# nrlugg/fenix

Measured on AMD Instinct MI355X. Metric: vectors/sec + %HBM roofline, 10M×768 f32 L2 kNN k=100 at 1/2/4/8 GPU, higher is better.
Workload: dtype f32; 1 GPU; 10Mx768 f32 L2 kNN k=100, single query, per GPU; rows_per_gpu=10000000, total_rows=10000000, d=768, k=100, queries=1, metric=l2, parallelism=row-shard x1, one process per GPU

## Files before the change

fenix_amd/_lib.py:

```python

from __future__ import annotations

import contextlib
import ctypes
import hashlib
import os
import threading
from typing import Iterator

HERE = os.path.dirname(os.path.abspath(__file__))
LIB_PATH = os.environ.get("FENIX_AMD_LIB") or os.path.join(HERE, "lib", "libfenix_knn.so")

DTYPE_F32 = 0
DTYPE_F16 = 1
DTYPE_QU8 = 2
METRIC_L2 = 0
METRIC_IP = 1
METRIC_COS = 2

METRICS = {
    "l2": METRIC_L2,
    "euclidean": METRIC_L2,
    "inner_product": METRIC_IP,
    "dot": METRIC_IP,
    "cosine": METRIC_COS,
}

SYMBOLS = (
    "fx_version",
    "fx_last_error",
    "fx_device_count",
    "fx_max_k",
    "fx_knn_workspace_bytes",
    "fx_knn_workspace_bytes_img8",
    "fx_knn_search",
    "fx_knn_scan",
    "fx_knn_reduce",
    "fx_filter_image_bytes",
    "fx_filter_image",
    "fx_filter_image_used",
    "fx_knn_scan_img",
    "fx_knn_search_img",
    "fx_filter_image8_bytes",
    "fx_filter_image8",
    "fx_knn_scan_img8",
    "fx_knn_search_img8",
    "fx_knn_reduce_img8",
    "fx_filter_image8_typed",
    "fx_filter_image8_perm",
    "fx_knn_filter_counts",
    "fx_knn_filter_state",
    "fx_knn_distances",
    "fx_topk_merge_workspace_bytes",
    "fx_topk_merge",
    "fx_fill_normal",
    "fx_row_sqnorms",
    "fx_code_assign_workspace_bytes",
    "fx_code_assign",
    "fx_kmeans_step_workspace_bytes",
    "fx_kmeans_step",
    "fx_code_assign_ex",
    "fx_kmeans_step_ex",
    "fx_code_probe_workspace_bytes",
    "fx_code_probe",
    "fx_code_mask",
    "fx_code_qmask_workspace_bytes",
    "fx_code_qmask",
    "fx_knn_search_rows_workspace_bytes",
    "fx_knn_search_rows",
    "fx_mask_compact_workspace_bytes",
    "fx_mask_compact",
    "fx_pred_limits",
    "fx_pred_eval",
    "fx_knn_search_ex_workspace_bytes",
    "fx_knn_search_ex",
    "fx_knn_search_shards_workspace_bytes",
    "fx_knn_search_shards",
    "fx_knn_distances_ex",
    "fx_filter_image8_ex",
    "fx_knn_scan_img8_ex",
    "fx_knn_reduce_img8_ex",
    "fx_knn_search_img8_ex",
    "fx_qmask_words",
    "fx_qmask_pack",
    "fx_qmask_filter_used",
    "fx_knn_scan_qmask_ex",
    "fx_knn_reduce_qmask_ex",
    "fx_knn_search_qmask_ex",
    "fx_comm_init_all",
    "fx_comm_destroy",
    "fx_allgather_topk",
    "fx_set_option",
    "fx_get_option",
    "fx_host_sync_count",
)

OPTIONS = ("batched", "batch_min_queries", "batch_cap", "batch_sample_ratio", "force_fallback",
           "scan_interleave", "q8_dma", "filter_image", "batch_ub_test", "single_query_image",
           "i8_max_k", "img6", "img8", "i8_sample_ratio", "i8_grow_ratio", "select_prune",
           "scan_stream", "filter_hold", "qu8_batch_min_work", "qmask_batch_min_ratio",
           "device_filter_min_rows")

_lock = threading.Lock()
_lib = None


class Corpus(ctypes.Structure):

    _fields_ = [
        ("data", ctypes.c_void_p),
        ("dtype", ctypes.c_int),
        ("n", ctypes.c_int64),
        ("d", ctypes.c_int64),
        ("row_base", ctypes.c_int64),
        ("scale", ctypes.c_float),
        ("zero_point", ctypes.c_int32),
    ]


class PredColumn(ctypes.Structure):

    _fields_ = [
        ("values", ctypes.c_void_p),
        ("valid", ctypes.c_void_p),
        ("dtype", ctypes.c_int32),
        ("reserved", ctypes.c_int32),
    ]


class PredOp(ctypes.Structure):

    _fields_ = [
        ("op", ctypes.c_int32),
        ("column", ctypes.c_int32),
        ("imm", ctypes.c_int64),
        ("set_offset", ctypes.c_int32),
        ("set_length", ctypes.c_int32),
    ]


class FenixHipError(RuntimeError):
    """A HIP runtime failure inside the kNN engine."""


def load() -> ctypes.CDLL:
    global _lib
    with _lock:
        if _lib is not None:
            return _lib
        if not os.path.exists(LIB_PATH):
            raise ImportError(
                f"fenix_amd HIP library not built: {LIB_PATH} is missing "
                "(run __graft_entry__.build() or `make -C fenix_amd/csrc`)"
            )
        L = ctypes.CDLL(LIB_PATH)
        i64, sz, vp, ci = ctypes.c_int64, ctypes.c_size_t, ctypes.c_void_p, ctypes.c_int
        L.fx_version.argtypes = []
        L.fx_version.restype = ci
        L.fx_last_error.argtypes = []
        L.fx_last_error.restype = ctypes.c_char_p
        L.fx_device_count.argtypes = [ctypes.POINTER(ci)]
        L.fx_device_count.restype = ci
        L.fx_max_k.argtypes = []
        L.fx_max_k.restype = i64
        L.fx_knn_workspace_bytes.argtypes = [i64, i64, ci, i64, i64, ctypes.POINTER(sz)]
        L.fx_knn_workspace_bytes.restype = ci
        L.fx_knn_workspace_bytes_img8.argtypes = [i64, i64, ci, i64, i64, ci, ctypes.POINTER(sz)]
        L.fx_knn_workspace_bytes_img8.restype = ci
        L.fx_knn_search.argtypes = [vp, ci, i64, i64, i64, vp, i64, ci, i64, vp, vp, sz, vp, vp,
                                    vp]
        L.fx_knn_search.restype = ci
        L.fx_knn_scan.argtypes = [vp, ci, i64, i64, i64, vp, i64, ci, i64, vp, vp, sz, vp]
        L.fx_knn_scan.restype = ci
        L.fx_knn_reduce.argtypes = [vp, ci, i64, i64, i64, vp, i64, ci, i64, vp, vp, sz, vp, vp,
                                    vp]
        L.fx_knn_reduce.restype = ci
        L.fx_filter_image_bytes.argtypes = [i64, i64, ctypes.POINTER(sz), ctypes.POINTER(sz)]
        L.fx_filter_image_bytes.restype = ci
        L.fx_filter_image.argtypes = [vp, i64, i64, vp, vp, vp]
        L.fx_filter_image.restype = ci
        L.fx_filter_image_used.argtypes = [i64, i64, ci, i64, i64, ci, ctypes.POINTER(ci)]
        L.fx_filter_image_used.restype = ci
        L.fx_knn_scan_img.argtypes = [vp, ci, i64, i64, i64, vp, vp, vp, i64, ci, i64, vp, vp, sz,
                                      vp]
        L.fx_knn_scan_img.restype = ci
        L.fx_knn_search_img.argtypes = [vp, ci, i64, i64, i64, vp, vp, vp, i64, ci, i64, vp, vp,
                                        sz, vp, vp, vp]
        L.fx_knn_search_img.restype = ci
        L.fx_filter_image8_bytes.argtypes = [i64, i64, ctypes.POINTER(sz), ctypes.POINTER(sz)]
        L.fx_filter_image8_bytes.restype = ci
        L.fx_filter_image8.argtypes = [vp, i64, i64, vp, vp, vp]
        L.fx_filter_image8.restype = ci
        L.fx_filter_image8_typed.argtypes = [vp, ci, i64, i64, vp, vp, vp]
        L.fx_filter_image8_typed.restype = ci
        L.fx_filter_image8_perm.argtypes = [i64, ctypes.POINTER(ctypes.c_uint64)]
        L.fx_filter_image8_perm.restype = ci
        L.fx_knn_filter_counts.argtypes = [vp, ci, i64, i64, i64, ci, i64, ci, vp, sz, vp,
                                           ctypes.POINTER(i64), vp]
        L.fx_knn_filter_counts.restype = ci
        L.fx_knn_filter_state.argtypes = [vp, ci, i64, i64, i64, ci, i64, ci, vp, sz, vp, vp, vp,
                                          vp]
        L.fx_knn_filter_state.restype = ci
        L.fx_knn_scan_img8.argtypes = L.fx_knn_scan_img.argtypes
        L.fx_knn_scan_img8.restype = ci
        L.fx_knn_search_img8.argtypes = L.fx_knn_search_img.argtypes
        L.fx_knn_search_img8.restype = ci
        L.fx_knn_reduce_img8.argtypes = [vp, ci, i64, i64, i64, vp, vp, i64, ci, i64, vp, vp, sz,
                                         vp, vp, vp]
        L.fx_knn_reduce_img8.restype = ci
        L.fx_knn_distances.argtypes = [vp, ci, i64, i64, vp, i64, ci, vp, vp, vp]
        L.fx_knn_distances.restype = ci
        L.fx_topk_merge_workspace_bytes.argtypes = [i64, i64, i64, i64, ctypes.POINTER(sz)]
        L.fx_topk_merge_workspace_bytes.restype = ci
        L.fx_topk_merge.argtypes = [vp, vp, i64, i64, i64, i64, vp, sz, vp, vp, vp]
        L.fx_topk_merge.restype = ci
        L.fx_fill_normal.argtypes = [vp, ci, i64, i64, ctypes.c_uint64, i64, i64, vp]
        L.fx_fill_normal.restype = ci
        L.fx_row_sqnorms.argtypes = [vp, ci, i64, i64, vp, vp]
        L.fx_row_sqnorms.restype = ci
        psz = ctypes.POINTER(sz)
        L.fx_code_assign_workspace_bytes.argtypes = [i64, i64, i64, i64, psz]
        L.fx_code_assign_workspace_bytes.restype = ci
        L.fx_code_assign.argtypes = [vp, ci, i64, i64, vp, i64, i64, ci, vp, sz, vp, vp, vp, vp]
        L.fx_code_assign.restype = ci
        L.fx_kmeans_step_workspace_bytes.argtypes = [i64, i64, i64, i64, psz]
        L.fx_kmeans_step_workspace_bytes.restype = ci
        L.fx_kmeans_step.argtypes = [vp, ci, i64, i64, i64, vp, i64, ci, vp, sz, vp]
        L.fx_kmeans_step.restype = ci
        L.fx_code_assign_ex.argtypes = [ctypes.POINTER(Corpus), vp, i64, i64, ci, vp, sz, vp, vp,
                                        vp, vp]
        L.fx_code_assign_ex.restype = ci
        L.fx_kmeans_step_ex.argtypes = [ctypes.POINTER(Corpus), i64, vp, i64, ci, vp, sz, vp]
        L.fx_kmeans_step_ex.restype = ci
        L.fx_code_probe_workspace_bytes.argtypes = [i64, i64, i64, psz]
        L.fx_code_probe_workspace_bytes.restype = ci
        L.fx_code_probe.argtypes = [vp, i64, i64, i64, i64, vp, sz, vp, vp, vp, vp]
        L.fx_code_probe.restype = ci
        L.fx_code_mask.argtypes = [vp, i64, vp, i64, vp, vp, vp, vp]
        L.fx_code_mask.restype = ci
        L.fx_code_qmask_workspace_bytes.argtypes = [i64, i64, psz]
        L.fx_code_qmask_workspace_bytes.restype = ci
        L.fx_code_qmask.argtypes = [vp, i64, vp, i64, i64, i64, vp, vp, sz, vp, i64, vp, vp, vp]
        L.fx_code_qmask.restype = ci
        L.fx_knn_search_rows_workspace_bytes.argtypes = [i64, i64, ci, i64, i64, psz]
        L.fx_knn_search_rows_workspace_bytes.restype = ci
        L.fx_knn_search_rows.argtypes = [vp, ci, i64, i64, i64, vp, i64, vp, i64, ci, i64, vp, sz,
                                         vp, vp, vp]
        L.fx_knn_search_rows.restype = ci
        L.fx_mask_compact_workspace_bytes.argtypes = [i64, psz]
        L.fx_mask_compact_workspace_bytes.restype = ci
        L.fx_mask_compact.argtypes = [vp, i64, vp, sz, vp, vp, vp]
        L.fx_mask_compact.restype = ci
        pi = ctypes.POINTER(ci)
        L.fx_pred_limits.argtypes = [pi, pi, pi, pi]
# ... 266 lines not shown
```

fenix_amd/csrc/filter/tiled.inc:

```
#ifndef FX_I3_SEG
#define FX_I3_SEG 24
#endif
typedef __attribute__((address_space(3))) void* i3_lds_ptr;

template <int N>
__device__ __forceinline__ void i3_wait_barrier() {
  asm volatile("s_waitcnt vmcnt(%0)\n\ts_waitcnt lgkmcnt(0)\n\ts_barrier" ::"n"(N) : "memory");
}

__device__ __forceinline__ uint32_t lds_add_rtn_u32(uint32_t* p, uint32_t v) {
  const uint32_t a = (uint32_t)(uintptr_t)(__attribute__((address_space(3))) uint32_t*)(p);
  uint32_t r;
  asm volatile("ds_add_rtn_u32 %0, %1, %2\n\ts_waitcnt lgkmcnt(0)" : "=v"(r) : "v"(a), "v"(v) : "memory");
  return r;
}
__device__ __forceinline__ void lds_write1_u32(uint32_t* p, uint32_t x) {
  const uint32_t a = (uint32_t)(uintptr_t)(__attribute__((address_space(3))) uint32_t*)(p);
  asm volatile("ds_write_b32 %0, %1" ::"v"(a), "v"(x) : "memory");
}
__device__ __forceinline__ void lds_write2_u32(uint2* p, uint32_t x, uint32_t y) {
  const uint32_t a = (uint32_t)(uintptr_t)(__attribute__((address_space(3))) uint2*)(p);
  asm volatile("ds_write_b64 %0, %1" ::"v"(a), "v"(uint2{x, y}) : "memory");
}
__device__ __forceinline__ void lds_write3_u32(uint32_t* p, uint32_t x, uint32_t y, uint32_t z) {
  const uint32_t a = (uint32_t)(uintptr_t)(__attribute__((address_space(3))) uint32_t*)(p);
  asm volatile("ds_write_b32 %0, %1\n\tds_write_b32 %0, %2 offset:4\n\tds_write_b32 %0, %3 offset:8"
               ::"v"(a), "v"(x), "v"(y), "v"(z) : "memory");
}

constexpr float kI8Magic = 12582912.f;
constexpr float kI8C0 = 12582912.f - 8.f;

template <int METRIC>
__device__ __forceinline__ void i8_query_table(const FilterArgs& a, int64_t q0, f32x4* qtab,
                                               f32x4* qinf, int tid, int nthreads) {
  const float u = 5.9604644775390625e-08f;
  const float g = (float)(a.d + 2) * u * 1.01f;
  for (int i = tid; i < fBQ; i += nthreads) {
    const int64_t gq = q0 + i;
    f32x4 c = f32x4(0.f), qi = f32x4(0.f);
    if (gq < a.nq) {
      qi = *reinterpret_cast<const f32x4*>(a.qinfo + gq * kI8QInfo);
      float tf = key_float((uint32_t)(a.thr[gq] >> 32));
      if (a.ub_test) tf += fabsf(tf) * 6.103515625e-05f;
      const float sq = qi[0];
      c[0] = qi[1];
      if constexpr (METRIC == 1) {
        const float t = tf / sq;
        c[1] = t + 16.f * u * fabsf(t);
      } else if constexpr (METRIC == 2) {
        const float cc = 3.f * g + 16.f * u;
        const float K = (1.f - 2.f * tf - 2.f * cc) * (fmaxf(qi[3], 1e-12f) / sq);
        c[1] = -K + (g + 16.f * u) * fabsf(K);
      } else {
        const float g2 = 2.f * g + 8.f * u;
        const float L1 = 0.5f / sq;
        const float t2 = tf * tf * (1.f + 9.5367431640625e-07f) / (1.f - g2);
        const float L0 = (qi[2] * (1.f - 4.f * u) - t2) * L1;
        c[1] = -L1 * (1.f - g - 16.f * u);
        c[2] = -L0 + 16.f * u * fabsf(L0);
      }
      if (tf != tf || !(c[0] <= 3.4e38f))
        c = f32x4{__builtin_inff(), 0.f, 0.f, 0.f};
      else if (a.ub_test)
        c[0] = -c[0];
    }
    qtab[i] = c;
    qinf[i] = qi;
  }
}

template <int METRIC>
__device__ __forceinline__ void i8_bounds(float m, float om, float y1, float is, f32x4 qi, int d,
                                          float& lb, float& ub) {
  if (om != om) {
    lb = -__builtin_inff();
    ub = __builtin_nanf("");
    return;
  }
  const float u = 5.9604644775390625e-08f;
  const float g = (float)(d + 2) * u * 1.01f;
  const float I = m - kI8Magic;
  const float E = fmaf(om * qi[1], 8.f * u, om * qi[1]) + 4.f;
  const float s = 1.f / is;
  const float sig = s * qi[0];
  const float a1 = I + E, a2 = I - E;
  if constexpr (METRIC == 1) {
    const float lo = -sig * a1, hi = -sig * a2;
    lb = lo - 16.f * u * fabsf(lo);
    ub = hi + 16.f * u * fabsf(hi);
  } else if constexpr (METRIC == 2) {
    const float c = 3.f * g + 32.f * u;
    const float den = fmaxf(y1 * s, 1e-12f) * fmaxf(qi[3], 1e-12f);
    const float r1 = sig * a1 / den, r2 = sig * a2 / den;
    lb = 0.5f - 0.5f * r1 - c - 16.f * u * (1.f + fabsf(r1));
    ub = 0.5f - 0.5f * r2 + c + 16.f * u * (1.f + fabsf(r2));
  } else {
    const float g2 = 2.f * g + 8.f * u;
    const float n2 = y1 * s;
    const float alo = n2 * (1.f - g - 16.f * u) + qi[2] * (1.f - 4.f * u);
    const float ahi = n2 * (1.f + g + 16.f * u) + qi[2] * (1.f + 4.f * u);
    const float t1 = 2.f * sig * a1, t2 = 2.f * sig * a2;
    const float lo2 = (1.f - g2) * (alo - t1) - 16.f * u * (alo + fabsf(t1));
    const float hi2 = (1.f + g2) * (ahi - t2) + 16.f * u * (ahi + fabsf(t2));
    lb = sqrtf(fmaxf(lo2, 0.f)) * (1.f - 4.f * u);
    ub = sqrtf(fmaxf(hi2, 0.f)) * (1.f + 4.f * u);
  }
  if (lb != lb) lb = -__builtin_inff();
  if (ub != ub) ub = __builtin_nanf("");
}

__device__ __forceinline__ void i8_note_row(float* rinfo, float* rterm, float* rext,
                                            uint32_t* flags, int lr, float om, float y1, float is,
                                            bool ok) {
  rinfo[lr] = om;
  rterm[lr] = y1;
  rext[lr] = is;
  int word, bit;
  filter_row_bit<1>(lr, word, bit);
  if (!ok) atomicOr(&flags[16 + word], 1u << bit);
  else if (om != om) atomicOr(&flags[word], 1u << bit);
}

constexpr int64_t kAllPassSlotTiles = 64;
template <int METRIC, bool QMASK = false>
__device__ __forceinline__ void i8_epilogue(const f32x16 (&acc)[kI2QT], const float* rinfo,
                                            const float* rterm, const float* rext,
                                            const uint32_t* rrow, const uint32_t* flags,
                                            const f32x4* qtab, const f32x4* qinf,
                                            const FilterArgs& a, int64_t q0, int wid, int h,
                                            int l32, uint32_t* seg, int diag,
                                            int segcap = FX_I3_SEG,
                                            const uint32_t* rqmask = nullptr) {
  const int lr0 = wid * 32 + 4 * h;
  const uint32_t fmask = flags[wid * 2 + h], smask = flags[16 + wid * 2 + h];
  uint32_t fail[kI2QT];
#pragma unroll
  for (int u = 0; u < kI2QT; ++u) fail[u] = 0u;
  const f32x2 nc0 = {-kI8C0, -kI8C0};
#pragma unroll
  for (int g = 3; g >= 0; --g) {
    const f32x4 om = *reinterpret_cast<const f32x4*>(rinfo + lr0 + 8 * g);
    const f32x4 y1 = *reinterpret_cast<const f32x4*>(rterm + lr0 + 8 * g);
    f32x4 y2 = f32x4(0.f);
    if constexpr (METRIC == 0) y2 = *reinterpret_cast<const f32x4*>(rext + lr0 + 8 * g);
#pragma unroll
    for (int u = 0; u < kI2QT; ++u) {
      const f32x4 co = qtab[u * 32 + l32];
      const f32x2 ra = {co[0], co[0]}, c1 = {co[1], co[1]}, c2 = {co[2], co[2]};
#pragma unroll
      for (int hp = 1; hp >= 0; --hp) {
        const int i = 2 * g + hp;
        const f32x2 xp = {acc[u][2 * i], acc[u][2 * i + 1]};
        const f32x2 op = hp ? f32x2{om[2], om[3]} : f32x2{om[0], om[1]};
        const f32x2 p1 = hp ? f32x2{y1[2], y1[3]} : f32x2{y1[0], y1[1]};
        f32x2 t = __builtin_elementwise_fma(op, ra, xp);
        t = __builtin_elementwise_fma(p1, c1, t);
        if constexpr (METRIC == 0) {
          const f32x2 p2 = hp ? f32x2{y2[2], y2[3]} : f32x2{y2[0], y2[1]};
          t = __builtin_elementwise_fma(p2, c2, t);
        }
        const f32x2 dd = t + nc0;
        fail[u] = __builtin_amdgcn_alignbit(fail[u], __float_as_uint(dd[1]), 31);
        fail[u] = __builtin_amdgcn_alignbit(fail[u], __float_as_uint(dd[0]), 31);
      }
    }
  }
  uint32_t pm[kI2QT];
  const uint32_t force = a.all_pass ? ~0u : fmask;
  uint32_t qbits[kI2QT];
#pragma unroll
  for (int u = 0; u < kI2QT; ++u) qbits[u] = 0xffffu;
  if constexpr (QMASK) {
    typedef uint32_t qw_t __attribute__((ext_vector_type(kI2QT)));
#pragma unroll
    for (int u = 0; u < kI2QT; ++u) qbits[u] = 0u;
#pragma unroll
    for (int j = 0; j < 16; ++j) {
      const qw_t w = reinterpret_cast<const qw_t*>(rqmask)[lr0 + (j & 3) + 8 * (j >> 2)];
#pragma unroll
      for (int u = 0; u < kI2QT; ++u) qbits[u] |= ((w[u] >> l32) & 1u) << j;
    }
  }
#pragma unroll
  for (int u = 0; u < kI2QT; ++u) {
    pm[u] = (diag & 1) ? 0u : (~fail[u] | force) & ~smask & qbits[u] & 0xffffu;
    if (q0 + u * 32 + l32 >= a.nq) pm[u] = 0u;
  }
  if (a.all_pass && (segcap <= FX_I3_SEG || a.num_tiles <= kAllPassSlotTiles)) {
    static_for<kI2QT>([&](auto uc) {
      constexpr int u = decltype(uc)::value;
      const uint32_t bits = pm[u];
      if (__ballot(bits != 0u) == 0ull) return;
      const int qi = u * 32 + (int)opaque((unsigned)l32);
      const int64_t gq = q0 + qi;
      uint32_t p = bits != 0u ? atomicAdd(&a.count[gq * kCountStride], (uint32_t)__popc(bits)) : 0u;
      const f32x4 qrec = qinf[qi];
      static_for<16>([&](auto jc) {
        constexpr int jj = decltype(jc)::value;
        if (!((bits >> jj) & 1u)) return;
        const int lr = (int)opaque((unsigned)lr0) + (jj & 3) + 8 * (jj >> 2);
        float lb, ub;
        i8_bounds<METRIC>(acc[u][jj], rinfo[lr], rterm[lr], rext[lr], qrec, a.d, lb, ub);
        if (p < (uint32_t)a.cap) {
          const uint32_t grow = rrow[lr];
          const size_t slot = (size_t)gq * a.cap + p;
          if (a.cand_ub != nullptr) {
            a.cand[slot] = make_comp(lb, grow);
            a.cand_ub[slot] = make_comp(ub, grow);
          } else {
            a.cand[slot] = make_comp(ub, grow);
          }
        }
        ++p;
      });
    });
    return;
  }
  uint32_t any = 0u;
#pragma unroll
  for (int u = 0; u < kI2QT; ++u) any |= pm[u];
  if (__ballot(any != 0u) == 0ull) return;
  static_for<kI2QT>([&](auto uc) {
    constexpr int u = decltype(uc)::value;
    if (__ballot(pm[u] != 0u) == 0ull) return;
    const int qi = u * 32 + (int)opaque((unsigned)l32);
    const int64_t gq = q0 + qi;
// ... 46 lines not shown
```

fenix_amd/csrc/fx_internal.h:

```cpp
#pragma once

#include "../../include/fenix_knn.h"
#include "fx_common.h"

namespace fx {

constexpr int kModeTopk = 0;
constexpr int kModeDist = 1;
constexpr int kCountStride = 32;
constexpr int kSelectMaxK = 2048;

#define FX_OPTIONS(FX_OPTION)                               \
  FX_OPTION(kOptBatched, "batched", 1)                      \
  FX_OPTION(kOptBatchMinQ, "batch_min_queries", 2)          \
  FX_OPTION(kOptBatchCap, "batch_cap", 0)                   \
  FX_OPTION(kOptBatchRatio, "batch_sample_ratio", 0)        \
  FX_OPTION(kOptForceFallback, "force_fallback", 0)         \
  FX_OPTION(kOptScanInterleave, "scan_interleave", -1)      \
  FX_OPTION(kOptQ8Dma, "q8_dma", 1)                         \
  FX_OPTION(kOptFilterImage, "filter_image", 8)             \
  FX_OPTION(kOptBatchUbTest, "batch_ub_test", 1)            \
  FX_OPTION(kOptSingleImage, "single_query_image", 1)       \
  FX_OPTION(kOptI8MaxK, "i8_max_k", 1024)                   \
  FX_OPTION(kOptImg6, "img6", 1)                            \
  FX_OPTION(kOptImg8, "img8", 1)                            \
  FX_OPTION(kOptI8SampleRatio, "i8_sample_ratio", 8)        \
  FX_OPTION(kOptI8GrowRatio, "i8_grow_ratio", 16)           \
  FX_OPTION(kOptSelectPrune, "select_prune", 1)             \
  FX_OPTION(kOptScanStream, "scan_stream", -1)             \
  FX_OPTION(kOptFilterHold, "filter_hold", 0)               \
  FX_OPTION(kOptQu8BatchMinWork, "qu8_batch_min_work", 204800000) \
  FX_OPTION(kOptQmaskBatchMinRatio, "qmask_batch_min_ratio", 123) \
  FX_OPTION(kOptDeviceFilterMinRows, "device_filter_min_rows", 10000)
enum Option : int {
#define FX_OPTION_ENUM(id, name, dflt) id,
  FX_OPTIONS(FX_OPTION_ENUM)
#undef FX_OPTION_ENUM
  kOptCount
};
int64_t option(Option o);
int set_option(const char* name, int64_t value);
int get_option(const char* name, int64_t* out);
const char* last_error();

#ifdef FX_DIAG_BUILD
int diag_env(const char* name, int dflt);
#else
constexpr int diag_env(const char*, int dflt) { return dflt; }
#endif

struct ScanArgs {
  const void* X;
  int64_t n;
  int d;
  int64_t row_base;
  const float* q;
  const uint32_t* mask;
  const int32_t* rows;
  int64_t rows_per_block;
  int k;
  int cap;
  size_t qbytes;
  int mode;
  uint64_t* out_lists;
  int64_t list_stride;
  int64_t list_base;
  float* out_dist;
  float qscale, qshift;
  int interleave;
  int mask_qstride;
  const uint32_t* gate;
  int64_t gate_cap;
};

typedef void (*ScanKernelFn)(ScanArgs);

struct ScanPlan {
  ScanKernelFn fn;
  int W, L, U, cap;
  size_t qbytes, smem;
  int64_t blocks, rows_per_block, nlists;
  int interleave;
  ScanKernelFn fn_plain;
  size_t smem_plain;
  const char* plain_name;
};

int plan_scan(int64_t n, int64_t d, int dtype, int64_t k, int metric, bool aligned, ScanPlan* p);
void limit_scan_blocks(ScanPlan* p, int64_t n, int64_t max_blocks);
int launch_scan(const ScanPlan& p, const ScanArgs& a, int64_t nq, hipStream_t stream);

struct MergePlan {
  int levels;
  int64_t group[16];
  int64_t lists[17];
  int64_t klen[17];
  size_t ws_bytes;
};
int plan_merge(int64_t nq, int64_t nlists, int64_t kin, int64_t k, MergePlan* p);
int run_merge(const MergePlan& p, const uint64_t* in, int64_t nq, int64_t k, void* ws,
              float* out_dist, int64_t* out_row, hipStream_t stream,
              uint64_t* out_kth = nullptr, const uint32_t* gate = nullptr,
              int64_t gate_cap = 0, uint32_t* count = nullptr, bool zero_count = false);

struct Quant {
  float scale = 1.f, shift = 0.f;
};

template <typename F>
int for_query_chunks(int64_t nq, F&& f) {
  for (int64_t q0 = 0; q0 < nq; q0 += 65535) {
    if (int rc = f(q0, (nq - q0) < 65535 ? (nq - q0) : 65535)) return rc;
  }
  return FX_OK;
}

struct ExactSource {
  const void* X;
  int dtype;
  int64_t n;
  int d;
  int64_t row_base;
  const float* Q;
  const float* qnorm;
  int metric;
  Quant z;
  ExactSource from_query(int64_t q0) const {
    ExactSource s = *this;
    s.Q += q0 * d;
    if (s.qnorm != nullptr) s.qnorm += q0;
    return s;
  }
};

int launch_qu8_query(const float* Q, int64_t nq, int d, Quant z, float* out, hipStream_t stream);
int launch_qnorm(const float* Q, int64_t nq, int d, float* out, hipStream_t stream);
int launch_rescore(const ExactSource& src, int64_t nq, const uint32_t* count, uint64_t* cand,
                   int cap, const uint64_t* thr, hipStream_t stream);
int launch_exact_kth(const ExactSource& src, int64_t nq, int k, int64_t* rows, uint64_t* thr,
                     hipStream_t stream);

struct PruneScratch {
  uint64_t* lists = nullptr;
  int count = 0;
  bool on() const { return lists != nullptr && count > 0; }
  uint64_t* from_query(int64_t q0, int k) const {
    return on() ? lists + q0 * (int64_t)count * k : nullptr;
  }
};
int select_prune_lists(int64_t k, int64_t cap);
size_t select_prune_bytes(int64_t nq, int64_t k, int prune_lists);
struct OverflowGate {
  const uint64_t* cand = nullptr;
  int64_t num = 0, den = 1;
};
int launch_exact_threshold(const ExactSource& src, int64_t nq, const uint64_t* keys, int64_t cap,
                           uint32_t* count, bool zero_count, int k, uint64_t* thr,
                           PruneScratch prune, int64_t* topr, OverflowGate gate,
                           hipStream_t stream);
int launch_sample_threshold(const uint64_t* keys, int64_t nq, int64_t cap, uint32_t* count,
                            bool zero_count, int k, uint64_t* thr, PruneScratch prune,
                            hipStream_t stream);
int launch_final_select(const uint64_t* keys, int64_t nq, int64_t cap, const uint32_t* count,
                        int k, float* out_dist, int64_t* out_row, const uint64_t* alt,
                        int64_t alt_m, int64_t alt_gate, PruneScratch prune, hipStream_t stream);

struct FilterArgs {
  const void* X;
  int dtype;
  int64_t n;
  int d;
  int64_t row_base;
  const uint16_t* Qh;
  int dq;
  int64_t qstride;
  const float* qinfo;
  int64_t nq;
  const uint32_t* mask;
  int64_t tile_start, tile_stride, num_tiles;
  const uint64_t* thr;
  uint32_t* count;
  uint64_t* cand;
  uint64_t* cand_ub;
  int cap;
  const float* rowinfo;
  int img8;
// ... 59 lines not shown
```

fenix_amd/csrc/knn_filter.hip:

```cpp
#include "fx_internal.h"

namespace fx {
namespace q256 {
int launch(const FilterArgs& a, int metric, hipStream_t stream);
}
namespace q64 {
int launch(const FilterArgs& a, int metric, hipStream_t stream);
}
namespace q128 {
int launch(const FilterArgs& a, int metric, hipStream_t stream);
int launch_img6(const FilterArgs& a, int metric, hipStream_t stream);
bool img6_fits(int dq);
bool img6_fits_qmask(int dq);
}
namespace q64i {
int launch(const FilterArgs& a, int metric, hipStream_t stream);
int launch_img6(const FilterArgs& a, int metric, hipStream_t stream);
bool img6_fits(int dq);
bool img6_fits_qmask(int dq);
}
namespace h256 {
int launch(const FilterArgs& a, int metric, hipStream_t stream);
}

bool image_tiled() { return diag_env("FX_IMAGE_TILED", 1) != 0; }

bool filter_ring() { return diag_env("FX_FILTER_RING", 0) != 0; }

int launch_filter(const FilterArgs& a, int metric, hipStream_t stream) {
  if (a.qmask != nullptr) {
    const int kind = a.img8 ? filter_qmask_kind(a.dq, a.nq) : 0;
    if (kind == 0) {
      set_error("filter: per-query masks need an int8 image whose query slice fits (dq=%d)", a.dq);
      return FX_EUNSUPPORTED;
    }
    return kind == 128 ? q128::launch_img6(a, metric, stream) : q64i::launch_img6(a, metric, stream);
  }
  if (a.img8) {
    const int64_t i6 = option(kOptImg6);
    if (a.nq <= 64) {
      if (i6 >= 1 && q64i::img6_fits(a.dq)) return q64i::launch_img6(a, metric, stream);
      return q64i::launch(a, metric, stream);
    }
    if (a.nq <= 128) {
      if (i6 >= 1 && q128::img6_fits(a.dq)) return q128::launch_img6(a, metric, stream);
      return q128::launch(a, metric, stream);
    }
    if (i6 >= 2 && q128::img6_fits(a.dq)) return q128::launch_img6(a, metric, stream);
    return q256::launch(a, metric, stream);
  }
  if (a.nq <= 64) return q64::launch(a, metric, stream);
  if (a.nq <= 128 && !filter_ring()) return q128::launch(a, metric, stream);
  if (a.rowinfo != nullptr && image_tiled()) return q256::launch(a, metric, stream);
  if (a.dtype == FX_DTYPE_F16 && !filter_ring()) return h256::launch(a, metric, stream);
  return q256::launch(a, metric, stream);
}

int filter_qmask_kind(int dq, int64_t nq) {
  if (nq > 64 && q128::img6_fits_qmask(dq)) return 128;
  return q64i::img6_fits_qmask(dq) ? 64 : 0;
}

int filter_tile_rows(int dtype) {
  (void)dtype;
  return kFilterTileRows;
}

int filter_query_pad(int64_t nq) { return nq <= 64 ? 64 : nq <= 128 && !filter_ring() ? 128 : 256; }
int filter_dq(int d) { return (d + 63) / 64 * 64; }

__global__ void qprep_kernel(const float* __restrict__ Q, int64_t nq, int64_t nq_pad, int d, int dq,
                             int metric, uint16_t* __restrict__ Qh, float* __restrict__ qinfo) {
  const int64_t q = (int64_t)blockIdx.x * 4 + (threadIdx.x >> 6);
  const int lane = threadIdx.x & 63;
  if (q >= nq_pad) return;
  _Float16* out = reinterpret_cast<_Float16*>(Qh) + q * 32;
  auto at = [&](int i) -> _Float16& { return out[(int64_t)(i >> 5) * nq_pad * 32 + (i & 31)]; };
  if (q >= nq) {
    for (int i = lane; i < dq; i += 64) at(i) = (_Float16)0.f;
    return;
  }
  const float* qv = Q + q * (int64_t)d;
  float s = 0.f, m = 0.f;
  for (int i = lane; i < d; i += 64) {
    s = fmaf(qv[i], qv[i], s);
    m = fmaxf(m, fabsf(qv[i]));
  }
#pragma unroll
  for (int o = 32; o >= 1; o >>= 1) {
    s += __shfl_xor(s, o);
    m = fmaxf(m, __shfl_xor(m, o));
  }
  int ex = 0;
  if (m > 0.f && m <= 3.4e38f) (void)frexpf(m, &ex);
  const int sh = 15 - ex;
  const float scale = ldexpf(1.f, sh > 126 ? 126 : (sh < -126 ? -126 : sh));
  for (int i = lane; i < dq; i += 64) at(i) = (_Float16)(i < d ? qv[i] * scale : 0.f);
  if (lane == 0) {
    const double u = 1.0 / 2048.0, g = 5.9604644775390625e-08;
    const double sd = sqrt((double)d);
    const double rel = 1.25 * (2.0 * u + u * u + sd * 1.4901161193847656e-08 + (4.0 * d + 16.0) * g);
    const double abs_ = 1.25 * sd * 6.103515625e-05 * (1.0 + 1.0 / 1024.0);
    const float qn = sqrtf(s);
    float a, b, t;
    if (metric == FX_METRIC_L2) {
      t = s;
      a = (float)rel;
      b = (float)(2.0 * abs_ * (double)qn);
    } else if (metric == FX_METRIC_IP) {
      t = qn;
      a = (float)(rel * (double)qn);
      b = (float)(abs_ * (double)qn);
    } else {
      t = fmaxf(qn, 1e-12f);
      a = (float)(0.5 * rel);
      b = (float)(0.5 * abs_);
    }
    if (!(s <= 3.4e38f) || !(m <= 3.4e38f)) a = __builtin_inff();
    float* info = qinfo + q * 4;
    info[0] = 1.f / scale;
    info[1] = t;
    info[2] = a;
    info[3] = b;
  }
}

int launch_qprep(const float* Q, int64_t nq, int64_t nq_pad, int d, int dq, int metric,
                 uint16_t* Qh, float* qinfo, hipStream_t stream) {
  hipLaunchKernelGGL(qprep_kernel, dim3((unsigned)((nq_pad + 3) / 4)), dim3(256), 0, stream, Q,
                     nq, nq_pad, d, dq, metric, Qh, qinfo);
  return check_launch("qprep_kernel");
}

typedef float img_f32x4 __attribute__((ext_vector_type(4)));
typedef _Float16 img_f16x4 __attribute__((ext_vector_type(4)));
#ifdef FX_DIAG_BUILD
__global__ void __launch_bounds__(256) image_kernel(const float* __restrict__ X, int64_t n, int d,
                                                    _Float16* __restrict__ img,
                                                    float* __restrict__ rowinfo) {
  const int lane = threadIdx.x & 63;
  const int64_t nw = (int64_t)gridDim.x * 4;
  for (int64_t r = (int64_t)blockIdx.x * 4 + (threadIdx.x >> 6); r < n; r += nw) {
    const img_f32x4* xr = reinterpret_cast<const img_f32x4*>(X + r * d);
    img_f16x4* ir = reinterpret_cast<img_f16x4*>(img + r * d);
    float s = 0.f, m = 0.f;
    for (int i = lane; i < d / 4; i += 64) {
      const img_f32x4 v = __builtin_nontemporal_load(xr + i);
      ir[i] = __builtin_convertvector(v, img_f16x4);
#pragma unroll
      for (int e = 0; e < 4; ++e) {
        s = fmaf(v[e], v[e], s);
        m = fmaxf(m, fabsf(v[e]));
      }
    }
#pragma unroll
    for (int o = 32; o >= 1; o >>= 1) {
      s += __shfl_xor(s, o);
      m = fmaxf(m, __shfl_xor(m, o));
    }
    if (lane == 0) rowinfo[r] = (s <= 3.4e38f && m < 65520.f) ? s : __builtin_nanf("");
  }
}
#endif

typedef _Float16 img_f16x8 __attribute__((ext_vector_type(8)));
__global__ void __launch_bounds__(256) image_tiled_kernel(const float* __restrict__ X, int64_t n,
                                                          int d, _Float16* __restrict__ img,
                                                          float* __restrict__ rowinfo) {
  const int lane = threadIdx.x & 63, h = lane >> 5;
  const int64_t nt = (n + 31) / 32;
  const int ksteps = (d + 15) / 16;
  const int64_t nw = (int64_t)gridDim.x * 4;
  for (int64_t t = (int64_t)blockIdx.x * 4 + (threadIdx.x >> 6); t < nt; t += nw) {
    const int64_t r = t * 32 + (lane & 31);
    const bool live = r < n;
    const float* xr = X + (live ? r : 0) * (int64_t)d;
    img_f16x8* out = reinterpret_cast<img_f16x8*>(img) + t * ksteps * 64 + lane;
    float s = 0.f, m = 0.f;
#pragma unroll 4
    for (int ks = 0; ks < ksteps; ++ks) {
      const int k0 = 16 * ks + 8 * h;
      const bool ok = live && k0 < d;
      const float* p = xr + (k0 < d ? k0 : 0);
      img_f32x4 a = *reinterpret_cast<const img_f32x4*>(p);
      img_f32x4 b = *reinterpret_cast<const img_f32x4*>(p + 4);
      if (!ok) {
        a = img_f32x4(0.f);
        b = img_f32x4(0.f);
      }
#pragma unroll
      for (int e = 0; e < 4; ++e) {
// ... 359 lines not shown
```

fenix_amd/csrc/knn_filter_q64i.hip:

```cpp
#include "fx_internal.h"

#include <type_traits>

#define FX_FILTER_BQ 64
#define FX_FILTER_BK 32

namespace fx {
namespace q64i {

#include "filter/tile.inc"
#include "filter/tiled.inc"
#include "filter/img3.inc"
#include "filter/img6.inc"
#ifdef FX_DIAG_BUILD
#include "filter/ring.inc"
#endif

int launch(const FilterArgs& a, int metric, hipStream_t stream) {
  if (a.num_tiles <= 0) return FX_OK;
  if (a.rowinfo != nullptr && image_tiled())
    return launch_img3(a, metric, stream);
#ifdef FX_DIAG_BUILD
  if (filter_ring()) return launch_ring_rows(a, metric, stream);
#endif
  set_error("filter: row type not compiled into this variant");
  return FX_EUNSUPPORTED;
}

}
}
```

Measured before the change: 2.321 billion vectors/s.

## Add register-ring int8 filter kernel for one or two queries

After: 2.321 billion vectors/s (median of 2 runs). Within noise of the previous version (-0.0%).

```diff
diff --git a/fenix_amd/_lib.py b/fenix_amd/_lib.py
--- a/fenix_amd/_lib.py
+++ b/fenix_amd/_lib.py
@@ -99,7 +99,7 @@
            "scan_interleave", "q8_dma", "filter_image", "batch_ub_test", "single_query_image",
            "i8_max_k", "img6", "img8", "i8_sample_ratio", "i8_grow_ratio", "select_prune",
            "scan_stream", "filter_hold", "qu8_batch_min_work", "qmask_batch_min_ratio",
-           "device_filter_min_rows")
+           "device_filter_min_rows", "img1")
 
 _lock = threading.Lock()
 _lib = None
diff --git a/fenix_amd/csrc/filter/img1.inc b/fenix_amd/csrc/filter/img1.inc
--- /dev/null
+++ b/fenix_amd/csrc/filter/img1.inc
@@ -0,0 +1,257 @@
+#ifndef FX_I1_RING
+#define FX_I1_RING 6
+#endif
+#ifndef FX_I1_BLOCKS
+#define FX_I1_BLOCKS 1
+#endif
+#ifndef FX_I1_LOCKSTEP
+#define FX_I1_LOCKSTEP 0
+#endif
+#ifndef FX_I1_SEG
+#define FX_I1_SEG 32
+#endif
+constexpr int kI1Waves = 8;
+constexpr int kI1Threads = 64 * kI1Waves;
+constexpr int kI1MaxQ = 2;
+static_assert(32 * kI1Waves == fBM, "a workgroup's waves cover one plan tile per step");
+static_assert(FX_I1_SEG >= 32, "a segment takes one sub-tile's passes");
+struct Img1Shared {
+  f32x4 qtab[fBQ];
+  f32x4 qinf[fBQ];
+  uint32_t seg[kI1Waves][kI1MaxQ][3 * FX_I1_SEG];
+};
+static int img1_qbytes(int d, int dq) {
+  const int ksteps = (d + 31) / 32;
+  const int nks = (ksteps + FX_I1_RING - 1) / FX_I1_RING * FX_I1_RING;
+  return nks * 32 > dq ? nks * 32 : dq;
+}
+
+template <int METRIC, int NQ>
+__global__ void __launch_bounds__(kI1Threads, FX_I1_BLOCKS) filter_img1_kernel(FilterArgs a) {
+  constexpr int R = FX_I1_RING, SEG = FX_I1_SEG;
+  extern __shared__ __attribute__((aligned(16))) unsigned char smem[];
+  Img1Shared* sh = reinterpret_cast<Img1Shared*>(smem);
+  unsigned char* qs = smem + sizeof(Img1Shared);
+  const int tid = threadIdx.x, lane = tid & 63;
+  const int wid = __builtin_amdgcn_readfirstlane(tid >> 6);
+  const int h = lane >> 5, l32 = lane & 31;
+  const int ksteps = (a.d + 31) / 32;
+  const int ngroups = (ksteps + R - 1) / R;
+  const int qbytes = ngroups * R * 32 > a.dq ? ngroups * R * 32 : a.dq;
+  const int64_t ntile32 = (a.n + 31) / 32;
+  const int64_t nsub = a.num_tiles * kI1Waves;
+  const int64_t gstep = (int64_t)gridDim.x * kI1Waves;
+  int64_t s = (int64_t)blockIdx.x * kI1Waves + wid;
+  if (a.skip_full) {
+    bool full = true;
+#pragma unroll
+    for (int q = 0; q < NQ; ++q)
+      if (a.count[q * kCountStride] <= (uint32_t)a.cap) full = false;
+    if (__syncthreads_and(full)) return;
+  }
+  auto sub_t32 = [&](int64_t s) {
+    return (a.tile_start + (s >> 3) * a.tile_stride) * kI1Waves + (s & 7);
+  };
+  struct Desc {
+    uint32_t lo, hi;
+    int nb;
+  };
+  auto x_desc = [&](int64_t s) {
+    const int64_t t32 = sub_t32(s);
+    const int64_t live = (s < nsub && t32 < ntile32) ? 1 : 0;
+    const unsigned char* base = reinterpret_cast<const unsigned char*>(a.X) +
+                                (live ? t32 : 0) * (int64_t)ksteps * 1024;
+    const uint64_t xp = reinterpret_cast<uint64_t>(base);
+    Desc d;
+    d.lo = __builtin_amdgcn_readfirstlane((uint32_t)xp);
+    d.hi = __builtin_amdgcn_readfirstlane((uint32_t)(xp >> 32));
+    d.nb = __builtin_amdgcn_readfirstlane((int)(live * ksteps * 1024));
+    return d;
+  };
+  auto x_rsrc = [&](const Desc& d) {
+    return __builtin_amdgcn_make_buffer_rsrc(
+        reinterpret_cast<void*>(((uint64_t)d.hi << 32) | d.lo), 0, d.nb, 0x00020000);
+  };
+  const uint32_t xl = (uint32_t)opaque(lane) * 16u;
+  auto load_a = [&](__amdgpu_buffer_rsrc_t xr, int ks) {
+    const uint32_t off = ks < ksteps ? xl : 0x7fff0000u;
+    return __builtin_bit_cast(i32x4, __builtin_amdgcn_raw_buffer_load_b128(xr, off, ks * 1024, 2));
+  };
+  struct Terms {
+    f32x4 rsum;
+    uint32_t crow, mword;
+    bool in;
+  };
+  auto load_terms = [&](int64_t s) {
+    Terms t;
+    const int64_t row = sub_t32(s) * 32 + l32;
+    t.in = s < nsub && row < a.n;
+    const int64_t rowc = t.in ? row : a.n - 1;
+    t.crow = perm_row(a.perm_a, a.n, rowc);
+    t.rsum = *reinterpret_cast<const f32x4*>(a.rowinfo + rowc * kI8RowInfo);
+    const uint32_t* mp = a.mask != nullptr ? a.mask + (t.crow >> 5)
+                                           : reinterpret_cast<const uint32_t*>(a.rowinfo + rowc * kI8RowInfo);
+    t.mword = *mp;
+    return t;
+  };
+  Desc xr = x_desc(s);
+  i32x4 xa[R];
+#pragma unroll
+  for (int i = 0; i < R; ++i) xa[i] = load_a(x_rsrc(xr), i);
+  Terms cur = load_terms(s);
+  i8_query_table<METRIC>(a, 0, sh->qtab, sh->qinf, tid, kI1Threads);
+  {
+    const unsigned char* qb = reinterpret_cast<const unsigned char*>(a.Qh);
+    const int pieces = qbytes / 16;
+    for (int i = tid; i < NQ * pieces; i += kI1Threads) {
+      const int q = i / pieces, o = (i % pieces) * 16;
+      i32x4 v = i32x4(0);
+      if (o < a.dq)
+        v = *reinterpret_cast<const i32x4*>(qb + ((int64_t)(o >> 6) * a.qstride + q) * 64 + (o & 63));
+      *reinterpret_cast<i32x4*>(qs + q * qbytes + o) = v;
+    }
+  }
+  __syncthreads();
+  const int qsel = NQ == 2 ? h : 0;
+  const f32x4 co = sh->qtab[qsel];
+  const f32x4 qrec = sh->qinf[qsel];
+  const unsigned char* qlane = qs + h * 16;
+  uint32_t cnt[NQ];
+#pragma unroll
+  for (int q = 0; q < NQ; ++q) cnt[q] = 0u;
+  auto flush = [&](int q, uint32_t n) {
+    uint32_t base = 0u;
+    if (lane == 0) base = atomicAdd(&a.count[q * kCountStride], n);
+    base = __builtin_amdgcn_readfirstlane(base);
+    const uint32_t* e0 = sh->seg[wid][q];
+    for (uint32_t j = (uint32_t)lane; j < n; j += 64u) {
+      const uint32_t p = base + j;
+      if (p >= (uint32_t)a.cap) continue;
+      const uint32_t* e = e0 + 3 * j;
+      const size_t slot = (size_t)q * a.cap + p;
+      if (a.cand_ub != nullptr) {
+        a.cand[slot] = ((uint64_t)e[0] << 32) | e[2];
+        a.cand_ub[slot] = ((uint64_t)e[1] << 32) | e[2];
+      } else {
+        a.cand[slot] = ((uint64_t)e[1] << 32) | e[2];
+      }
+    }
+  };
+  const int acc0 = h == 0 ? (int)__float_as_uint(kI8Magic) : 0;
+  for (; s < nsub; s += gstep) {
+    const int64_t sn = s + gstep;
+    const Desc xn = x_desc(sn);
+    const Terms nxt = load_terms(sn);
+    int acc[NQ];
+#pragma unroll
+    for (int q = 0; q < NQ; ++q) acc[q] = acc0;
+    int g = 0;
+    do {
+      const bool last = g + 1 == ngroups;
+      const unsigned char* qg = qlane + g * (R * 32);
+      Desc xf;
+      xf.lo = last ? xn.lo : xr.lo;
+      xf.hi = last ? xn.hi : xr.hi;
+      xf.nb = last ? xn.nb : xr.nb;
+      const __amdgpu_buffer_rsrc_t xs = x_rsrc(xf);
+      const int kb = last ? 0 : (g + 1) * R;
+      i32x4 qv[NQ][R];
+#pragma unroll
+      for (int q = 0; q < NQ; ++q)
+#pragma unroll
+        for (int i = 0; i < R; ++i)
+          qv[q][i] = *reinterpret_cast<const i32x4*>(qg + q * qbytes + i * 32);
+      __builtin_amdgcn_sched_barrier(0);
+#pragma unroll
+      for (int i = 0; i < R; ++i) {
+#pragma unroll
+        for (int q = 0; q < NQ; ++q)
+#pragma unroll
+          for (int e = 0; e < 4; ++e)
+            acc[q] = __builtin_amdgcn_sdot4(xa[i][e], qv[q][i][e], acc[q], false);
+        __builtin_amdgcn_sched_barrier(0);
+        xa[i] = load_a(xs, kb + i);
+        __builtin_amdgcn_sched_barrier(0);
+      }
+    } while (++g < ngroups);
+    int tot;
+    if constexpr (NQ == 2) {
+      const int give = h ? acc[0] : acc[1], keep = h ? acc[1] : acc[0];
+      tot = keep + __shfl_xor(give, 32);
+    } else {
+      tot = acc[0] + __shfl_xor(acc[0], 32);
+    }
+    const float x = __uint_as_float((uint32_t)tot);
+    const float om = cur.rsum[0];
+    const float y1 = METRIC == 1 ? cur.rsum[1] : METRIC == 2 ? cur.rsum[2] : cur.rsum[3];
+    const float is = cur.rsum[1];
+    float t = __builtin_fmaf(om, co[0], x);
+    t = __builtin_fmaf(y1, co[1], t);
+    if constexpr (METRIC == 0) t = __builtin_fmaf(is, co[2], t);
+    const float dd = t + (-kI8C0);
+    const bool fail = (__float_as_uint(dd) >> 31) != 0u;
+    const bool ok = cur.in && (a.mask == nullptr || ((cur.mword >> (cur.crow & 31)) & 1u));
+    const bool pass = ok && (!fail || a.all_pass || om != om) && (NQ == 2 || h == 0);
+    const uint64_t bal = __ballot(pass);
+    if (bal != 0ull) {
+      float lb = 0.f, ub = 0.f;
+      if (pass) i8_bounds<METRIC>(x, om, y1, is, qrec, a.d, lb, ub);
+      const uint32_t grow = (uint32_t)a.row_base + cur.crow;
+#pragma unroll
+      for (int q = 0; q < NQ; ++q) {
+        const uint64_t mq = NQ == 2 ? (q ? bal & 0xffffffff00000000ull : bal & 0xffffffffull) : bal;
+        const uint32_t n = (uint32_t)__popcll(mq);
+        if (n == 0u) continue;
+        if (cnt[q] + n > (uint32_t)SEG) {
+          flush(q, cnt[q]);
+          cnt[q] = 0u;
+        }
+        const uint32_t rank = __builtin_amdgcn_mbcnt_hi(
+            (uint32_t)(mq >> 32), __builtin_amdgcn_mbcnt_lo((uint32_t)mq, 0u));
+        if (pass && qsel == q) {
+          uint32_t* e = sh->seg[wid][q] + 3 * (cnt[q] + rank);
+          e[0] = order_key(lb);
+          e[1] = order_key(ub);
+          e[2] = grow;
+        }
+        cnt[q] += n;
+      }
+    }
+    cur = nxt;
+    xr = xn;
+    if constexpr (FX_I1_LOCKSTEP != 0) __builtin_amdgcn_s_barrier();
+  }
+#pragma unroll
+  for (int q = 0; q < NQ; ++q)
+    if (cnt[q] != 0u) flush(q, cnt[q]);
+}
+
+bool img1_default(int d, int64_t nq) { return nq == 1 && (d + 31) / 32 == 24; }
+
+int launch_img1(const FilterArgs& a, int metric, hipStream_t stream) {
+  if (a.num_tiles <= 0) return FX_OK;
+  if (a.nq < 1 || a.nq > kI1MaxQ || a.qmask != nullptr || !a.img8) {
+    set_error("filter_img1_kernel: %lld queries (at most %d, no per-query masks)",
+              (long long)a.nq, kI1MaxQ);
+    return FX_EINVAL;
+  }
+  const bool two = a.nq == 2;
+  const void* fn =
+      two ? (metric == FX_METRIC_COS  ? (const void*)filter_img1_kernel<2, 2>
+             : metric == FX_METRIC_IP ? (const void*)filter_img1_kernel<1, 2>
+                                      : (const void*)filter_img1_kernel<0, 2>)
+          : (metric == FX_METRIC_COS  ? (const void*)filter_img1_kernel<2, 1>
+             : metric == FX_METRIC_IP ? (const void*)filter_img1_kernel<1, 1>
+                                      : (const void*)filter_img1_kernel<0, 1>);
+  const size_t smem = sizeof(Img1Shared) + (size_t)kI1MaxQ * img1_qbytes(a.d, a.dq);
+  if (smem > 64 * 1024) {
+    set_error("filter_img1_kernel: d=%d needs %zu bytes of LDS", a.d, smem);
+    return FX_EUNSUPPORTED;
+  }
+  int cus = 0;
+  if (int rc = device_cus(&cus)) return rc;
+  int64_t bx = (int64_t)cus * FX_I1_BLOCKS;
+  if (bx > a.num_tiles) bx = a.num_tiles;
+  return launch_query_tiles(fn, "filter_img1_kernel", a, kI1Threads, smem, bx, fBQ, kI8QInfo,
+                            stream);
+}
diff --git a/fenix_amd/csrc/filter/tiled.inc b/fenix_amd/csrc/filter/tiled.inc
--- a/fenix_amd/csrc/filter/tiled.inc
+++ b/fenix_amd/csrc/filter/tiled.inc
@@ -73,6 +73,7 @@
 template <int METRIC>
 __device__ __forceinline__ void i8_bounds(float m, float om, float y1, float is, f32x4 qi, int d,
                                           float& lb, float& ub) {
+#pragma clang fp contract(off)
   if (om != om) {
     lb = -__builtin_inff();
     ub = __builtin_nanf("");
diff --git a/fenix_amd/csrc/fx_internal.h b/fenix_amd/csrc/fx_internal.h
--- a/fenix_amd/csrc/fx_internal.h
+++ b/fenix_amd/csrc/fx_internal.h
@@ -31,7 +31,8 @@
   FX_OPTION(kOptFilterHold, "filter_hold", 0)               \
   FX_OPTION(kOptQu8BatchMinWork, "qu8_batch_min_work", 204800000) \
   FX_OPTION(kOptQmaskBatchMinRatio, "qmask_batch_min_ratio", 123) \
-  FX_OPTION(kOptDeviceFilterMinRows, "device_filter_min_rows", 10000)
+  FX_OPTION(kOptDeviceFilterMinRows, "device_filter_min_rows", 10000) \
+  FX_OPTION(kOptImg1, "img1", -1)
 enum Option : int {
 #define FX_OPTION_ENUM(id, name, dflt) id,
   FX_OPTIONS(FX_OPTION_ENUM)
diff --git a/fenix_amd/csrc/knn_filter.hip b/fenix_amd/csrc/knn_filter.hip
--- a/fenix_amd/csrc/knn_filter.hip
+++ b/fenix_amd/csrc/knn_filter.hip
@@ -18,6 +18,8 @@
 int launch_img6(const FilterArgs& a, int metric, hipStream_t stream);
 bool img6_fits(int dq);
 bool img6_fits_qmask(int dq);
+int launch_img1(const FilterArgs& a, int metric, hipStream_t stream);
+bool img1_default(int d, int64_t nq);
 }
 namespace h256 {
 int launch(const FilterArgs& a, int metric, hipStream_t stream);
@@ -37,6 +39,11 @@
     return kind == 128 ? q128::launch_img6(a, metric, stream) : q64i::launch_img6(a, metric, stream);
   }
   if (a.img8) {
+    if (a.nq <= 2) {
+      const int64_t i1 = option(kOptImg1);
+      if (i1 < 0 ? q64i::img1_default(a.d, a.nq) : i1 != 0)
+        return q64i::launch_img1(a, metric, stream);
+    }
     const int64_t i6 = option(kOptImg6);
     if (a.nq <= 64) {
       if (i6 >= 1 && q64i::img6_fits(a.dq)) return q64i::launch_img6(a, metric, stream);
diff --git a/fenix_amd/csrc/knn_filter_q64i.hip b/fenix_amd/csrc/knn_filter_q64i.hip
--- a/fenix_amd/csrc/knn_filter_q64i.hip
+++ b/fenix_amd/csrc/knn_filter_q64i.hip
@@ -12,6 +12,7 @@
 #include "filter/tiled.inc"
 #include "filter/img3.inc"
 #include "filter/img6.inc"
+#include "filter/img1.inc"
 #ifdef FX_DIAG_BUILD
 #include "filter/ring.inc"
 #endif
```
